# Harshs27/uGLAD

Measured on AMD Instinct MI355X. Metric: GLAD unroll-steps/sec (batch D×D Θ-updates), M=1024 D=128 L=30, higher is better.
Workload: dtype f32; 1 GPU; multi-task M=1024/GPU D=128 L=30 fp32 (BASELINE config 3; global batch 1024); pass=training step: forward + loss + backward + gradient exchange + Adam, sqrt_mode=ns10, parallelism=batch-sharded x1

## Files before the change

uglad_amd/csrc/glad_device.h:

```cpp
#pragma once
#include <hip/hip_runtime.h>

namespace uglad {

#ifndef UGLAD_THREADS
#define UGLAD_THREADS 512
#endif
constexpr int kThreads = UGLAD_THREADS;
constexpr int kWaves = kThreads / 64;
constexpr int kNsIters = 10;

constexpr int P_T = 0, P_RW1 = 1, P_RB1 = 10, P_RW2 = 13, P_RB2 = 22, P_RW3 = 25, P_RB3 = 28;
constexpr int P_LW1 = 29, P_LB1 = 35, P_LW2 = 38, P_LB2 = 41;
constexpr int kNParam = 42, kNRho = 28;

typedef float f32x16 __attribute__((ext_vector_type(16)));
struct alignas(16) f4 {
  float x, y, z, w;
};

#ifdef UGLAD_SIMT_EMUL
#define UGLAD_WAVE_SYNC() simt::wave_sync_point()
#else
#define UGLAD_WAVE_SYNC() asm volatile("s_waitcnt vmcnt(0) lgkmcnt(0)" ::: "memory")
#endif

template <int CTRL, int ROW_MASK = 0xf, int BANK_MASK = 0xf>
__device__ __forceinline__ float dpp_move(float v) {
  return __int_as_float(__builtin_amdgcn_update_dpp(0, __float_as_int(v), CTRL, ROW_MASK, BANK_MASK, false));
}

__device__ __forceinline__ float lane_xor1(float v) { return dpp_move<0xb1>(v); }

__device__ __forceinline__ float sum_halves(float v) {
#ifdef UGLAD_SIMT_EMUL
  return v + __shfl_xor(v, 32);
#else
  const auto r = __builtin_amdgcn_permlane32_swap(__float_as_uint(v), __float_as_uint(v), false, false);
  return __uint_as_float(r[0]) + __uint_as_float(r[1]);
#endif
}

__device__ __forceinline__ int opaque_v(int v) {
#ifndef UGLAD_SIMT_EMUL
  asm volatile("" : "+v"(v));
#endif
  return v;
}

template <typename T>
__device__ __forceinline__ T load_at(const float* __restrict__ base, unsigned bytes) {
  return *reinterpret_cast<const T*>(reinterpret_cast<const char*>(base) + bytes);
}

__device__ __forceinline__ float opaque_f(float v) {
#ifndef UGLAD_SIMT_EMUL
  asm volatile("" : "+v"(v));
#endif
  return v;
}

__device__ __forceinline__ int lane_now() {
#ifdef UGLAD_SIMT_EMUL
  return threadIdx.x & 63;
#else
  int l;
  asm volatile("v_mbcnt_lo_u32_b32 %0, -1, 0\n\tv_mbcnt_hi_u32_b32 %0, -1, %0" : "=v"(l));
  return l;
#endif
}

__device__ __forceinline__ float bcast_lane(float v, int src) {
  return __int_as_float(__builtin_amdgcn_readlane(__float_as_int(v), src));
}

__device__ __forceinline__ float wave_sum(float v) {
  v += dpp_move<0xb1>(v);
  v += dpp_move<0x4e>(v);
  v += dpp_move<0x124>(v);
  v += dpp_move<0x128>(v);
  v += dpp_move<0x142, 0xa>(v);
  v += dpp_move<0x143, 0xc>(v);
  return __int_as_float(__builtin_amdgcn_readlane(__float_as_int(v), 63));
}

__device__ __forceinline__ float block_sum(float v, float* s_red) {
  v = wave_sum(v);
  const int lane = threadIdx.x & 63, w = threadIdx.x >> 6;
  if (lane == 0) s_red[w] = v;
  __syncthreads();
  float t = 0.f;
#pragma unroll
  for (int i = 0; i < kWaves; ++i) t += s_red[i];
  __syncthreads();
  return t;
}

__device__ __forceinline__ float exp_acc(float x) {
  const float t = x * 1.44269504f;
  float e = fmaf(x, 1.44269504f, -t);
  e = fmaf(x, 1.925963033e-8f, e);
  const float r = __builtin_amdgcn_exp2f(t);
  return fmaf(r, e * 0.69314718f, r);
}

__device__ __forceinline__ float div_acc(float a, float b) {
  float q = __builtin_amdgcn_rcpf(b);
  q = fmaf(q, fmaf(-b, q, 1.0f), q);
  return a * q;
}

__device__ __forceinline__ float sigmoidf_(float x) {
  const float t = exp_acc(-fabsf(x));
  const float s = div_acc(1.0f, 1.0f + t);
  return (x >= 0.f) ? s : 1.0f - s;
}

__device__ __forceinline__ float tanhf_(float x) {
  const float t = exp_acc(-2.0f * fabsf(x));
  return copysignf(div_acc(1.0f - t, 1.0f + t), x);
}

struct RhoAct {
  float h1[3], h2[3], rho;
};

__device__ __forceinline__ void rho_forward(const float* __restrict__ p, float x1, float x2, float x3, RhoAct& a) {
#pragma unroll
  for (int o = 0; o < 3; ++o)
    a.h1[o] = tanhf_(fmaf(p[P_RW1 + 3 * o], x1, fmaf(p[P_RW1 + 3 * o + 1], x2, fmaf(p[P_RW1 + 3 * o + 2], x3, p[P_RB1 + o]))));
#pragma unroll
  for (int o = 0; o < 3; ++o)
    a.h2[o] = tanhf_(fmaf(p[P_RW2 + 3 * o], a.h1[0], fmaf(p[P_RW2 + 3 * o + 1], a.h1[1], fmaf(p[P_RW2 + 3 * o + 2], a.h1[2], p[P_RB2 + o]))));
  a.rho = sigmoidf_(fmaf(p[P_RW3], a.h2[0], fmaf(p[P_RW3 + 1], a.h2[1], fmaf(p[P_RW3 + 2], a.h2[2], p[P_RB3]))));
}

typedef float v2f __attribute__((ext_vector_type(2)));
__device__ __forceinline__ v2f fma2(v2f a, v2f b, v2f c) { return __builtin_elementwise_fma(a, b, c); }
__device__ __forceinline__ v2f splat2(float a) { return (v2f){a, a}; }
__device__ __forceinline__ v2f exp_acc2(v2f x) {
  const v2f t = x * 1.44269504f;
  v2f e = fma2(x, splat2(1.44269504f), -t);
  e = fma2(x, splat2(1.925963033e-8f), e);
  const v2f r = {__builtin_amdgcn_exp2f(t.x), __builtin_amdgcn_exp2f(t.y)};
  return fma2(r, e * 0.69314718f, r);
}
__device__ __forceinline__ v2f div_acc2(v2f a, v2f b) {
  v2f q = {__builtin_amdgcn_rcpf(b.x), __builtin_amdgcn_rcpf(b.y)};
  q = fma2(q, fma2(-b, q, splat2(1.0f)), q);
  return a * q;
}
__device__ __forceinline__ v2f tanh2(v2f x) {
  const v2f t = exp_acc2(-2.0f * __builtin_elementwise_abs(x));
  const v2f r = div_acc2(1.0f - t, 1.0f + t);
  return (v2f){copysignf(r.x, x.x), copysignf(r.y, x.y)};
}
__device__ __forceinline__ v2f sigmoid2(v2f x) {
  const v2f t = exp_acc2(-__builtin_elementwise_abs(x));
  const v2f s = div_acc2(splat2(1.0f), 1.0f + t);
  return (v2f){(x.x >= 0.f) ? s.x : 1.0f - s.x, (x.y >= 0.f) ? s.y : 1.0f - s.y};
}
struct RhoAct2 {
  v2f h1[3], h2[3], rho;
  __device__ __forceinline__ RhoAct half(int c) const {
    RhoAct a;
#pragma unroll
    for (int o = 0; o < 3; ++o) {
      a.h1[o] = c ? h1[o].y : h1[o].x;
      a.h2[o] = c ? h2[o].y : h2[o].x;
    }
    a.rho = c ? rho.y : rho.x;
    return a;
  }
};
__device__ __forceinline__ void rho_forward2(const float* __restrict__ p, v2f x1, v2f x2, v2f x3, RhoAct2& a) {
#pragma unroll
  for (int o = 0; o < 3; ++o)
    a.h1[o] = tanh2(fma2(splat2(p[P_RW1 + 3 * o]), x1,
                         fma2(splat2(p[P_RW1 + 3 * o + 1]), x2, fma2(splat2(p[P_RW1 + 3 * o + 2]), x3, splat2(p[P_RB1 + o])))));
#pragma unroll
  for (int o = 0; o < 3; ++o)
    a.h2[o] = tanh2(fma2(splat2(p[P_RW2 + 3 * o]), a.h1[0],
                         fma2(splat2(p[P_RW2 + 3 * o + 1]), a.h1[1], fma2(splat2(p[P_RW2 + 3 * o + 2]), a.h1[2], splat2(p[P_RB2 + o])))));
  a.rho = sigmoid2(fma2(splat2(p[P_RW3]), a.h2[0], fma2(splat2(p[P_RW3 + 1]), a.h2[1], fma2(splat2(p[P_RW3 + 2]), a.h2[2], splat2(p[P_RB3])))));
}

__device__ __forceinline__ float soft_threshold(float x, float rho) {
  const float m = fabsf(x) - rho;
  return m > 0.f ? copysignf(m, x) : 0.f;
}

__device__ __forceinline__ void rho_backward(const float* __restrict__ p, float x1, float x2, float x3, const RhoAct& a,
                                             float g_rho, float w, float* g, float& gx1, float& gx3) {
  const float go = g_rho * a.rho * (1.f - a.rho);
  const float gow = go * w;
  float ga2[3], ga1[3];
#pragma unroll
  for (int h = 0; h < 3; ++h) {
    g[(P_RW3 - 1) + h] += gow * a.h2[h];
    ga2[h] = go * p[P_RW3 + h] * (1.f - a.h2[h] * a.h2[h]);
  }
  g[P_RB3 - 1] += gow;
#pragma unroll
  for (int o = 0; o < 3; ++o) {
    const float t = ga2[o] * w;
#pragma unroll
    for (int h = 0; h < 3; ++h) g[(P_RW2 - 1) + 3 * o + h] += t * a.h1[h];
    g[(P_RB2 - 1) + o] += t;
  }
#pragma unroll
  for (int h = 0; h < 3; ++h) {
    const float s = ga2[0] * p[P_RW2 + h] + ga2[1] * p[P_RW2 + 3 + h] + ga2[2] * p[P_RW2 + 6 + h];
    ga1[h] = s * (1.f - a.h1[h] * a.h1[h]);
  }
#pragma unroll
  for (int o = 0; o < 3; ++o) {
    const float t = ga1[o] * w;
    g[(P_RW1 - 1) + 3 * o + 0] += t * x1;
    g[(P_RW1 - 1) + 3 * o + 1] += t * x2;
    g[(P_RW1 - 1) + 3 * o + 2] += t * x3;
    g[(P_RB1 - 1) + o] += t;
  }
  gx1 = ga1[0] * p[P_RW1 + 0] + ga1[1] * p[P_RW1 + 3] + ga1[2] * p[P_RW1 + 6];
  gx3 = ga1[0] * p[P_RW1 + 2] + ga1[1] * p[P_RW1 + 5] + ga1[2] * p[P_RW1 + 8];
}

__device__ __forceinline__ float rho_backward_col(const float* __restrict__ p, const RhoAct& a, float g_rho, int col) {
  const float go = g_rho * a.rho * (1.f - a.rho);
  float ga2[3], ga1[3];
#pragma unroll
  for (int h = 0; h < 3; ++h) ga2[h] = go * p[P_RW3 + h] * (1.f - a.h2[h] * a.h2[h]);
#pragma unroll
  for (int h = 0; h < 3; ++h) {
    const float s = ga2[0] * p[P_RW2 + h] + ga2[1] * p[P_RW2 + 3 + h] + ga2[2] * p[P_RW2 + 6 + h];
    ga1[h] = s * (1.f - a.h1[h] * a.h1[h]);
  }
  return ga1[0] * p[P_RW1 + col] + ga1[1] * p[P_RW1 + 3 + col] + ga1[2] * p[P_RW1 + 6 + col];
}

__device__ __forceinline__ void rho_backward2(const float* __restrict__ p, v2f x1, v2f x2, v2f x3, const RhoAct2& a, v2f g_rho,
                                              v2f w, v2f* g2, v2f& gx1, v2f& gx3) {
  const v2f go = g_rho * a.rho * (1.f - a.rho);
  const v2f gow = go * w;
  v2f ga2[3], ga1[3];
#pragma unroll
  for (int h = 0; h < 3; ++h) {
    g2[(P_RW3 - 1) + h] = fma2(gow, a.h2[h], g2[(P_RW3 - 1) + h]);
    ga2[h] = go * p[P_RW3 + h] * (1.f - a.h2[h] * a.h2[h]);
  }
  g2[P_RB3 - 1] += gow;
#pragma unroll
  for (int o = 0; o < 3; ++o) {
    const v2f t = ga2[o] * w;
#pragma unroll
    for (int h = 0; h < 3; ++h) g2[(P_RW2 - 1) + 3 * o + h] = fma2(t, a.h1[h], g2[(P_RW2 - 1) + 3 * o + h]);
    g2[(P_RB2 - 1) + o] += t;
  }
#pragma unroll
  for (int h = 0; h < 3; ++h) {
    const v2f s = ga2[0] * p[P_RW2 + h] + ga2[1] * p[P_RW2 + 3 + h] + ga2[2] * p[P_RW2 + 6 + h];
    ga1[h] = s * (1.f - a.h1[h] * a.h1[h]);
  }
#pragma unroll
  for (int o = 0; o < 3; ++o) {
    const v2f t = ga1[o] * w;
    g2[(P_RW1 - 1) + 3 * o + 0] = fma2(t, x1, g2[(P_RW1 - 1) + 3 * o + 0]);
    g2[(P_RW1 - 1) + 3 * o + 1] = fma2(t, x2, g2[(P_RW1 - 1) + 3 * o + 1]);
    g2[(P_RW1 - 1) + 3 * o + 2] = fma2(t, x3, g2[(P_RW1 - 1) + 3 * o + 2]);
    g2[(P_RB1 - 1) + o] += t;
  }
  gx1 = ga1[0] * p[P_RW1 + 0] + ga1[1] * p[P_RW1 + 3] + ga1[2] * p[P_RW1 + 6];
  gx3 = ga1[0] * p[P_RW1 + 2] + ga1[1] * p[P_RW1 + 5] + ga1[2] * p[P_RW1 + 8];
}

__device__ __forceinline__ float lambda_forward(const float* __restrict__ p, float n, float lam_prev) {
  float o = p[P_LB2];
#pragma unroll
  for (int h = 0; h < 3; ++h)
    o = fmaf(p[P_LW2 + h], tanhf(fmaf(p[P_LW1 + 2 * h], n, fmaf(p[P_LW1 + 2 * h + 1], lam_prev, p[P_LB1 + h]))), o);
  return sigmoidf_(o);
}

__device__ __forceinline__ float sqrt_spectrum(float beta, float c, float nrmA, int mode) {
  const float alpha = fmaf(beta, beta, c);
  if (mode == 0) return sqrtf(alpha);
  float y = alpha / nrmA, z = 1.f;
#pragma unroll
  for (int it = 0; it < kNsIters; ++it) {
    const float T = 0.5f * (3.f - z * y);
    y = y * T;
    z = T * z;
  }
  return y * sqrtf(nrmA);
}

__device__ __forceinline__ float shifted_spectrum(float be, int D, float lam, int mode, double* __restrict__ s3, float& alpha,
                                                  float& cond) {
  const int tid = threadIdx.x;
  const double c4 = 4.0 / (double)lam, b = (double)be;
  const double al = b * b + c4;
  const double r_exact = sqrt(al);
  if (tid < D) {
    s3[tid] = al * al;
    s3[D + tid] = 0.5 * (r_exact - b) * b;
    s3[2 * D + tid] = b * b;
  }
  __syncthreads();
  double* part = s3 + 3 * D;
  if ((tid >> 6) == 0) {
    const double* a = s3 + ((tid >> 4) < 3 ? (tid >> 4) : 2) * D;
    double s = 0.0, mx = 0.0, mn = 1e300;
    for (int i = tid & 15; i < D; i += 16) {
      const double v = a[i];
      s += v;
      mx = v > mx ? v : mx;
      mn = v < mn ? v : mn;
    }
#pragma unroll
    for (int o = 1; o < 16; o *= 2) {
      s += __shfl_xor(s, o);
      const double mxo = __shfl_xor(mx, o), mno = __shfl_xor(mn, o);
      mx = mxo > mx ? mxo : mx;
      mn = mno < mn ? mno : mn;
    }
    if ((tid & 15) == 0 && tid < 48) part[tid >> 4] = s;
    if (tid == 32) {
      part[3] = mx;
      part[4] = mn;
    }
  }
  __syncthreads();
  const double n2 = part[0], pb = part[1], bb = part[2], b2max = part[3], b2min = part[4];
  cond = (float)((b2max + c4) / (b2min + c4));
  double a_opt = (bb > 0.0) ? -pb / bb : 0.0;
  a_opt = a_opt < 0.0 ? 0.0 : (a_opt > 1.0 ? 1.0 : a_opt);
  alpha = (float)a_opt;
  double r = r_exact;
  if (mode != 0) {
    const double nrmA = sqrt(n2);
    double y = al / nrmA, z = 1.0;
#pragma unroll
    for (int it = 0; it < kNsIters; ++it) {
      const double T = 0.5 * (3.0 - z * y);
      y = y * T;
      z = T * z;
    }
    r = y * sqrt(nrmA);
  }
  const double psi = 0.5 * (r - b) + (double)alpha * b;
  __syncthreads();
  return (tid < D) ? (float)psi : 0.f;
}

template <int DP>
__device__ __forceinline__ void pair_of(int r, int k, int& i1, int& i2) {
  constexpr int m = DP - 1;
  if (k == 0) {
    i1 = m;
    i2 = r;
  } else {
    i1 = r + k;
    if (i1 >= m) i1 -= m;
    i2 = r + m - k;
    if (i2 >= m) i2 -= m;
  }
}

template <int DP>
__device__ void jacobi_eig(float* __restrict__ A, float* __restrict__ V, float* s_t, float* s_s, float* s_h, float* s_red,
                           int* s_flag) {
  constexpr int LD = DP + 1, H = DP / 2;
  const int tid = threadIdx.x;
  float fro = 0.f;
  for (int idx = tid; idx < DP * DP; idx += kThreads) {
    const float v = A[(idx / DP) * LD + (idx % DP)];
    fro = fmaf(v, v, fro);
  }
  fro = sqrtf(block_sum(fro, s_red));
  const float thresh = 1e-8f * fro;
  for (int sweep = 0; sweep < 16; ++sweep) {
    if (tid == 0) *s_flag = 0;
    __syncthreads();
    for (int r = 0; r < DP - 1; ++r) {
      if (tid < H) {
        int p, q;
        pair_of<DP>(r, tid, p, q);
        const float apq = A[p * LD + q];
        float t = 0.f, s = 0.f, h = 0.f;
        if (fabsf(apq) > thresh) {
          const float app = A[p * LD + p], aqq = A[q * LD + q];
          const float tau = (aqq - app) / (2.f * apq);
          t = copysignf(1.f, tau) / (fabsf(tau) + sqrtf(fmaf(tau, tau, 1.f)));
          const float c = 1.f / sqrtf(fmaf(t, t, 1.f));
          s = t * c;
          h = s / (1.f + c);
          *s_flag = 1;
        }
        s_t[tid] = t;
        s_s[tid] = s;
        s_h[tid] = h;
      }
      __syncthreads();
      for (int b = tid; b < H * H; b += kThreads) {
        const int kr = b / H, kc = b - kr * H;
        int r1, r2, c1, c2;
        pair_of<DP>(r, kr, r1, r2);
        pair_of<DP>(r, kc, c1, c2);
        const float x11 = A[r1 * LD + c1], x12 = A[r1 * LD + c2], x21 = A[r2 * LD + c1], x22 = A[r2 * LD + c2];
        float z11, z12, z21, z22;
        if (kr == kc) {
          const float t = s_t[kr];
          z11 = x11 - t * x12;
          z22 = x22 + t * x12;
          z12 = (t != 0.f) ? 0.f : x12;
          z21 = (t != 0.f) ? 0.f : x21;
        } else {
          const float sr = s_s[kr], hr = s_h[kr], sc = s_s[kc], hc = s_h[kc];
          const float y11 = x11 - sr * (x21 + hr * x11), y21 = x21 + sr * (x11 - hr * x21);
          const float y12 = x12 - sr * (x22 + hr * x12), y22 = x22 + sr * (x12 - hr * x22);
          z11 = y11 - sc * (y12 + hc * y11);
          z12 = y12 + sc * (y11 - hc * y12);
          z21 = y21 - sc * (y22 + hc * y21);
          z22 = y22 + sc * (y21 - hc * y22);
        }
        A[r1 * LD + c1] = z11;
        A[r1 * LD + c2] = z12;
        A[r2 * LD + c1] = z21;
        A[r2 * LD + c2] = z22;
      }
      for (int b = tid; b < DP * H; b += kThreads) {
        const int i = b / H, kc = b - i * H;
        int c1, c2;
        pair_of<DP>(r, kc, c1, c2);
        const float sc = s_s[kc], hc = s_h[kc];
        const float v1 = V[i * LD + c1], v2 = V[i * LD + c2];
        V[i * LD + c1] = v1 - sc * (v2 + hc * v1);
        V[i * LD + c2] = v2 + sc * (v1 - hc * v2);
      }
      __syncthreads();
    }
    if (*s_flag == 0) break;
    __syncthreads();
  }
  __syncthreads();
}

template <int NT, bool UPPER>
struct Tiles {
  static constexpr int kCount = UPPER ? NT * (NT + 1) / 2 : NT * NT;
  static constexpr int kPerWave = (kCount + kWaves - 1) / kWaves;
  __device__ static __forceinline__ void ij(int t, int& I, int& J) {
    if (UPPER) {
      int i = 0, rem = t;
      while (rem >= NT - i) {
        rem -= NT - i;
        ++i;
      }
      I = i;
      J = i + rem;
    } else {
      I = t / NT;
      J = t - I * NT;
    }
  }
};

__device__ __forceinline__ int acc_row(int reg, int lane) { return (reg & 3) + 8 * (reg >> 2) + 4 * (lane >> 5); }

__device__ __forceinline__ void mfma_tile(const float* __restrict__ Ap, int a_si, int a_sk, const float* __restrict__ Bp,
                                          int b_sk, int b_sj, int K, f32x16& acc) {
  const int lane = opaque_v(threadIdx.x) & 63, li = lane & 31, kh = lane >> 5;
  const float* a = Ap + li * a_si + kh * a_sk;
  const float* b = Bp + li * b_sj + kh * b_sk;
  float a0[8], b0[8], a1[8], b1[8];
#pragma unroll
  for (int u = 0; u < 8; ++u) {
    a0[u] = a[2 * u * a_sk];
    b0[u] = b[2 * u * b_sk];
  }
  for (int k = 0; k < K; k += 16) {
    const bool more = k + 16 < K;
    const float* an = a + (more ? 16 * a_sk : 0);
    const float* bn = b + (more ? 16 * b_sk : 0);
#pragma unroll
    for (int u = 0; u < 8; ++u) {
      a1[u] = an[2 * u * a_sk];
      b1[u] = bn[2 * u * b_sk];
    }
#pragma unroll
    for (int u = 0; u < 8; ++u) acc = __builtin_amdgcn_mfma_f32_32x32x2f32(a0[u], b0[u], acc, 0, 0, 0);
#pragma unroll
    for (int u = 0; u < 8; ++u) {
      a0[u] = a1[u];
      b0[u] = b1[u];
    }
    a = an;
    b = bn;
  }
}

#if defined(UGLAD_BF16X3) && !defined(UGLAD_SIMT_EMUL)
#include "../../scripts/retired/bf16x3_tile.h"
#define UGLAD_GEMM_TILE mfma_tile_bf16x3
#else
#define UGLAD_GEMM_TILE mfma_tile
#endif

template <int NT, bool TA, bool TB, bool UPPER>
__device__ __forceinline__ void gemm_lds(const float* __restrict__ X, const float* __restrict__ Y,
                                         f32x16 (&acc)[Tiles<NT, UPPER>::kPerWave]) {
  constexpr int DP = NT * 32, LD = DP + 1;
  using T = Tiles<NT, UPPER>;
  const int w = __builtin_amdgcn_readfirstlane(opaque_v(threadIdx.x) >> 6);
#pragma unroll
  for (int n = 0; n < T::kPerWave; ++n) {
    const int t = w + kWaves * n;
#pragma unroll
    for (int e = 0; e < 16; ++e) acc[n][e] = 0.f;
    if (t < T::kCount) {
      int I, J;
      T::ij(t, I, J);
      UGLAD_GEMM_TILE(TA ? X + I * 32 : X + I * 32 * LD, TA ? 1 : LD, TA ? LD : 1, TB ? Y + J * 32 * LD : Y + J * 32,
                      TB ? 1 : LD, TB ? LD : 1, DP, acc[n]);
    }
  }
}

template <int NT>
__device__ __forceinline__ void store_tiles(float* __restrict__ Y, const f32x16 (&acc)[Tiles<NT, false>::kPerWave]) {
  constexpr int LD = NT * 32 + 1;
  using T = Tiles<NT, false>;
  const int tid = opaque_v(threadIdx.x), lane = tid & 63, w = __builtin_amdgcn_readfirstlane(tid >> 6);
#pragma unroll
  for (int n = 0; n < T::kPerWave; ++n) {
    const int t = w + kWaves * n;
    if (t < T::kCount) {
      int I, J;
      T::ij(t, I, J);
#pragma unroll
      for (int e = 0; e < 16; ++e) Y[(I * 32 + acc_row(e, lane)) * LD + J * 32 + (lane & 31)] = acc[n][e];
    }
  }
}

#ifdef UGLAD_STAMPS
__device__ unsigned long long g_cwg[4096][3];
__device__ unsigned long long g_lstamps[4][96];
__device__ unsigned long long g_kstamps[32];
#define KSTAMP(i) do { if (threadIdx.x == 0 && blockIdx.x == 0) g_kstamps[i] = __builtin_amdgcn_s_memtime(); } while (0)
#define UGLAD_STAMP(ws, i) do { if (threadIdx.x == 0 && (i) < 64) (ws).stamp[i] = __builtin_amdgcn_s_memtime(); } while (0)
#elif defined(UGLAD_PHASE_EXIT)
__device__ int g_exit_at;
#define KSTAMP(i) do { if (g_exit_at == 100 + (i)) __builtin_amdgcn_endpgm(); } while (0)
#define UGLAD_STAMP(ws, i) do { if (g_exit_at == (i)) __builtin_amdgcn_endpgm(); } while (0)
#else
#define KSTAMP(i) do {} while (0)
#define UGLAD_STAMP(ws, i) do {} while (0)
#endif

__device__ __forceinline__ void copy_out_matrix(float* __restrict__ dst, const float* __restrict__ src, int D, int LD) {
  const int tid = threadIdx.x;
  if (((D & 3) == 0) && ((reinterpret_cast<size_t>(dst) & 15) == 0)) {
    const int D4 = D >> 2;
    for (int idx = tid; idx < D * D4; idx += kThreads) {
      const int i = idx / D4, j = 4 * (idx - i * D4);
      const float* p = src + i * LD + j;
      f4 v = {p[0], p[1], p[2], p[3]};
      *reinterpret_cast<f4*>(dst + (size_t)i * D + j) = v;
    }
  } else {
    const int si = kThreads / D, sj = kThreads - si * D;
    int i = tid / D, j = tid - i * D;
    for (int idx = tid; idx < D * D; idx += kThreads) {
      dst[idx] = src[i * LD + j];
      j += sj;
      i += si;
      if (j >= D) {
        j -= D;
        ++i;
      }
    }
  }
}

template <int DP>
constexpr int kTfacFloats = (DP / 32) * 1024;
template <int DP>
constexpr int kWsPerMatrix = 3 * DP + kTfacFloats<DP>;
template <int DP>
constexpr int big_floats() {
  return 2 * ((DP * (DP + 1) + 3) & ~3);
}
#define UGLAD_BIG_BUFFERS(A, NA, B, NB, GWS)                                                                     \
  constexpr bool kGM = DP > 128;                                                                                 \
  __shared__ __attribute__((aligned(16))) float A##_lds[kGM ? 4 : (NA)];                                         \
  __shared__ __attribute__((aligned(16))) float B##_lds[kGM ? 4 : (NB)];                                         \
  float* A = kGM ? (GWS) + (size_t)gridDim.x * kWsPerMatrix<DP> + (size_t)blockIdx.x * big_floats<DP>() : A##_lds; \
  float* B = kGM ? A + big_floats<DP>() / 2 : B##_lds;

template <int DP>
__device__ __forceinline__ float* tfac_behind_flags(float* ws, int M, int m) {
  static_assert(kTfacFloats<DP> / 2 >= 4, "flags and packed T factors outgrow the T region: M + 3 <= M kTfacFloats / 2 needs kTfacFloats / 2 >= 4");
  return ws + (size_t)M * 3 * DP + ((M + 3) & ~3) + (size_t)m * (kTfacFloats<DP> / 2);
}

}
```

uglad_amd/csrc/tridiag.h:

```cpp
#pragma once
#include "glad_device.h"

namespace uglad {

constexpr float kNegligibleSig = 1e-35f;

#ifdef UGLAD_STAMPS
__device__ unsigned long long g_tstamps[4];
__device__ unsigned long long g_twg[4096][3];
#define TSTAMP_BEGIN() const unsigned long long t_begin_ = __builtin_amdgcn_s_memtime()
#define TSTAMP_ADD(i) do { if (threadIdx.x == 0 && blockIdx.x == 0) g_tstamps[i] += __builtin_amdgcn_s_memtime() - t_begin_; } while (0)
#else
#define TSTAMP_BEGIN() do {} while (0)
#define TSTAMP_ADD(i) do {} while (0)
#endif

__device__ __forceinline__ float f4_elem(const f4& a, int q) { return q == 0 ? a.x : (q == 1 ? a.y : (q == 2 ? a.z : a.w)); }

template <int N>
__device__ __forceinline__ float pick(const float (&v)[N], int idx) {
  float r = v[0];
#pragma unroll
  for (int s = 1; s < N; ++s) r = (idx == s) ? v[s] : r;
  return r;
}

template <int NT, int TH>
__global__ __launch_bounds__(TH, NT <= 4 ? 8 : (TH > 512 ? 1 : 2)) void tridiag_kernel(const float* __restrict__ A0, const float* __restrict__ A1,
                                                           const float* __restrict__ lam_ptr, float* __restrict__ Rbase,
                                                           float* __restrict__ tri_base, int D, int gs,
                                                           const int* __restrict__ only_flagged) {
  if (only_flagged && only_flagged[blockIdx.x] == 0) return;
  constexpr int DP = NT * 32, RG = DP / 4, NCG = TH / RG, NC = (DP + NCG - 1) / NCG;
  constexpr int NS = (DP > 128) ? (DP + 63) / 64 : 2;
  constexpr int NL = (NT == 4 && TH == 512) ? 3 : 0;
  __shared__ f4 s_a[NL > 0 ? NL : 1][NL > 0 ? TH : 1];
  __shared__ __attribute__((aligned(16))) float s_vec[5 * DP];
#ifndef UGLAD_TRIDIAG_ROWWAVES
#define UGLAD_TRIDIAG_ROWWAVES 0
#endif
#ifndef UGLAD_TRIDIAG_PRIO
#define UGLAD_TRIDIAG_PRIO 1
#endif
#ifndef UGLAD_TRIDIAG_PAIRSUM
#define UGLAD_TRIDIAG_PAIRSUM 0
#endif
#ifndef UGLAD_TRIDIAG_LANE
#define UGLAD_TRIDIAG_LANE 0
#endif
#ifndef UGLAD_TRIDIAG_DPPSUM
#define UGLAD_TRIDIAG_DPPSUM 0
#endif
  constexpr bool kDppSum = UGLAD_TRIDIAG_DPPSUM && !UGLAD_TRIDIAG_ROWWAVES && (NT == 4 && TH == 512);
  constexpr bool kRowWaves = UGLAD_TRIDIAG_ROWWAVES && (NT == 4 && TH == 512);
  constexpr bool kPairSum = UGLAD_TRIDIAG_PAIRSUM && !kRowWaves && RG == 32 && (NCG % 2 == 0);
  constexpr int NPG = kDppSum ? 1 : (kPairSum ? NCG / 2 : NCG);
  constexpr int PS = kRowWaves ? DP + 4 : DP;
  __shared__ __attribute__((aligned(16))) float s_part[kRowWaves ? (TH / (DP / 4)) * (DP + 4) : TH * 4];
  __shared__ float s_dotp[(TH / 64)];
  __shared__ float s_corner, s_tau;
  const int tid = threadIdx.x, lane = tid & 63, wv = tid >> 6;
  const int wv_u = __builtin_amdgcn_readfirstlane(wv);
#ifdef UGLAD_STAMPS
  if (tid == 0 && blockIdx.x < 4096) {
    g_twg[blockIdx.x][0] = __builtin_amdgcn_s_memtime();
    unsigned hw, xcc;
    asm volatile("s_getreg_b32 %0, hwreg(HW_REG_HW_ID)" : "=s"(hw));
    asm volatile("s_getreg_b32 %0, hwreg(HW_REG_XCC_ID)" : "=s"(xcc));
    g_twg[blockIdx.x][2] = ((unsigned long long)xcc << 32) | hw;
  }
#endif
  const int r4 = kDppSum ? wv + 8 * (lane >> 4) : (kRowWaves ? 4 * wv + (lane & 3) : tid % RG);
  const int cg = kDppSum ? (lane & 15) : (kRowWaves ? lane >> 2 : tid / RG);
  const int cgw = (kRowWaves || kDppSum) ? NCG - 1 : (__builtin_amdgcn_readfirstlane(wv) * 64 + 63) / RG;
  const int cgmax = cgw < NCG - 1 ? cgw : NCG - 1;
  const int row_last = kRowWaves ? 16 * __builtin_amdgcn_readfirstlane(wv) + 15 : DP;
  const int n = D;
  const size_t base = (size_t)blockIdx.x * D * D;
  float* R = Rbase + base;
  float* tri = tri_base + (size_t)blockIdx.x * 3 * DP;
  const float inv_lam = lam_ptr ? 1.0f / lam_ptr[blockIdx.x / gs] : 1.0f;

  f4 a[NC];
  {
    auto pin = [](float v) { return opaque_f(v); };
    constexpr int LB = 4, LS = (NT == 3) ? 1 : 2;
    const float* __restrict__ Am = A0 + base;
    const float* __restrict__ Zm = A1 ? A1 + base : nullptr;
    const bool vec16 = !kDppSum && ((D & 3) == 0) && (((reinterpret_cast<size_t>(A0) | reinterpret_cast<size_t>(A1)) & 15) == 0);
    if (vec16) {
      const bool row_in = cg < NCG && 4 * r4 < n;
#pragma unroll
      for (int i0 = 0; i0 < NC; i0 += LB) {
        f4 s[LB], z[LB];
#pragma unroll
        for (int u = 0; u < LB; ++u) {
          const int c = cg + NCG * (i0 + u);
          const unsigned at = (i0 + u < NC && row_in && c < n) ? 4u * (c * D + 4 * r4) : 0u;
          s[u] = load_at<f4>(Am, at);
        }
        if (A1) {
#pragma unroll
          for (int u = 0; u < LB; ++u) {
            const int c = cg + NCG * (i0 + u);
            const unsigned at = (i0 + u < NC && row_in && c < n) ? 4u * (c * D + 4 * r4) : 0u;
            z[u] = load_at<f4>(Zm, at);
          }
          __builtin_amdgcn_sched_barrier(0);
        }
#pragma unroll
        for (int u = 0; u < LB; ++u) {
          const int i = i0 + u;
          if (i < NC) {
            const bool in = row_in && cg + NCG * i < n;
            f4 v = s[u];
            if (A1) v = {fmaf(inv_lam, v.x, -z[u].x), fmaf(inv_lam, v.y, -z[u].y), fmaf(inv_lam, v.z, -z[u].z), fmaf(inv_lam, v.w, -z[u].w)};
            a[i] = {pin(in ? v.x : 0.f), pin(in ? v.y : 0.f), pin(in ? v.z : 0.f), pin(in ? v.w : 0.f)};
            if (i < NL) s_a[i < NL ? i : 0][tid] = a[i];
          }
        }
      }
    } else {
#pragma unroll
      for (int i0 = 0; i0 < NC; i0 += LS) {
        float s[LS][4], z[LS][4];
#pragma unroll
        for (int u = 0; u < LS; ++u) {
          const int c = cg + NCG * (i0 + u);
#pragma unroll
          for (int q = 0; q < 4; ++q) {
            const int r = 4 * r4 + q;
            const bool in = i0 + u < NC && cg < NCG && c < n && r < n;
            const unsigned at = in ? 4u * (kDppSum ? r * D + c : c * D + r) : 0u;
            s[u][q] = load_at<float>(Am, at);
          }
        }
        if (A1) {
#pragma unroll
          for (int u = 0; u < LS; ++u) {
            const int c = cg + NCG * (i0 + u);
#pragma unroll
            for (int q = 0; q < 4; ++q) {
              const int r = 4 * r4 + q;
              const bool in = i0 + u < NC && cg < NCG && c < n && r < n;
              const unsigned at = in ? 4u * (kDppSum ? r * D + c : c * D + r) : 0u;
              z[u][q] = load_at<float>(Zm, at);
            }
          }
        }
#pragma unroll
        for (int u = 0; u < LS; ++u) {
          const int i = i0 + u;
          if (i < NC) {
            float t[4];
#pragma unroll
            for (int q = 0; q < 4; ++q) {
              const bool in = cg < NCG && cg + NCG * i < n && 4 * r4 + q < n;
              float v = s[u][q];
              if (A1) v = fmaf(inv_lam, v, -z[u][q]);
              t[q] = pin(in ? v : 0.f);
            }
            a[i] = {t[0], t[1], t[2], t[3]};
            if (i < NL) s_a[i < NL ? i : 0][tid] = a[i];
          }
        }
        __builtin_amdgcn_sched_barrier(0);
      }
    }
  }
  for (int i = tid; i < DP; i += TH) {
    s_vec[i] = 0.f;
    s_vec[DP + i] = 0.f;
    s_vec[2 * DP + i] = 0.f;
    tri[i] = 0.f;
    tri[DP + i] = 0.f;
    tri[2 * DP + i] = 0.f;
  }
  for (int i = tid; i < (int)(sizeof(s_part) / sizeof(float)); i += TH) s_part[i] = 0.f;
  if (tid < (TH / 64)) s_dotp[tid] = 0.f;
  if (cg == 0) *reinterpret_cast<f4*>(&s_vec[3 * DP + 4 * r4]) = a[0];
  if (cg < NCG && r4 == ((n - 1) >> 2)) {
#pragma unroll
    for (int i = 0; i < NC; ++i)
      if (cg + NCG * i == n - 1) s_corner = f4_elem(a[i], (n - 1) & 3);
  }
  __syncthreads();
  if (n == 1) {
    if (tid == 0) tri[0] = s_corner;
    return;
  }

#ifdef UGLAD_STAMPS
  if (tid == 0 && blockIdx.x == 0) g_tstamps[2] += __builtin_amdgcn_s_memtime() - g_twg[0][0];
#endif
  int ov = DP, on = 2 * DP;
  float tau_k = 0.f;
  int cur = 0;
  for (int k = -1; k <= n - 3; ++k) {
    const int k1 = k + 1;
    {
    TSTAMP_BEGIN();
    if (wv_u == 0) {
      if (UGLAD_TRIDIAG_PRIO) __builtin_amdgcn_s_setprio(3);
#if UGLAD_TRIDIAG_LANE == 1
      const int lane = lane_now();
      const int lane_k = lane;
#elif UGLAD_TRIDIAG_LANE == 2
      const int lane_k = lane_now();
#else
      const int lane_k = lane;
#endif
      float pv[NS], vv[NS], wl[NS];
#pragma unroll
      for (int s = 0; s < NS; ++s) {
        const int rr = lane_k + 64 * s;
        float p = 0.f;
        if (rr > k && lane + 64 * s < n) {
#pragma unroll 8
          for (int g = 0; g < NPG; ++g) p += s_part[g * PS + rr];
          p *= tau_k;
        }
        pv[s] = p;
        vv[s] = (lane + 64 * s < DP) ? s_vec[ov + rr] : 0.f;
      }
      float vAv2[2] = {0.f, 0.f};
#pragma unroll
      for (int q = 0; q < (TH / 64); ++q) vAv2[q & 1] += s_dotp[q];
      const float vAv = vAv2[0] + vAv2[1];
      const float alpha = 0.5f * tau_k * tau_k * vAv;
#pragma unroll
      for (int s = 0; s < NS; ++s) {
        const int rr = lane_k + 64 * s;
        wl[s] = pv[s] - alpha * vv[s];
        if (lane + 64 * s < DP) s_vec[rr] = wl[s];
      }
      const float w_k1 = bcast_lane(pick(wl, k1 >> 6), k1 & 63);
      const float v_k1 = bcast_lane(pick(vv, k1 >> 6), k1 & 63);
      float x[NS];
#pragma unroll
      for (int s = 0; s < NS; ++s) {
        const int c = lane_k + 64 * s;
        x[s] = (lane + 64 * s < n) ? (s_vec[(3 + cur) * DP + c] - v_k1 * wl[s] - w_k1 * vv[s]) : 0.f;
      }
      const float dk1 = bcast_lane(pick(x, k1 >> 6), k1 & 63);
      if (k1 <= n - 3) {
        const int c0 = k1 + 1;
        const float x0 = bcast_lane(pick(x, c0 >> 6), c0 & 63);
        float sig = 0.f;
#pragma unroll
        for (int s = 0; s < NS; ++s) {
          const int c = lane_k + 64 * s;
          if (c > c0 && lane + 64 * s < n) sig = fmaf(x[s], x[s], sig);
        }
        sig = wave_sum(sig);
        float beta = x0, tau1 = 0.f, sc = 0.f;
        if (sig > kNegligibleSig) {
          const float nrm2 = fmaf(x0, x0, sig);
          if (nrm2 > 1e-30f) {
            beta = -copysignf(__builtin_amdgcn_sqrtf(nrm2), x0);
            const float dd = x0 - beta;
            sc = div_acc(1.0f, dd);
            tau1 = -dd * div_acc(1.0f, beta);
          } else {
            beta = -copysignf(sqrtf(nrm2), x0);
            tau1 = (beta - x0) / beta;
            sc = 1.0f / (x0 - beta);
          }
        }
#pragma unroll
        for (int s = 0; s < NS; ++s) {
          const int c = lane_k + 64 * s;
          if (lane + 64 * s < DP) {
            float vc = 0.f;
            if (c == c0) vc = 1.f;
            else if (c > c0 && lane + 64 * s < n) vc = x[s] * sc;
            s_vec[on + c] = vc;
            if (lane + 64 * s < n) R[(size_t)k1 * D + c] = vc;
          }
        }
        if (lane == 0) {
          tri[k1] = dk1;
          tri[DP + k1] = beta;
          tri[2 * DP + k1] = tau1;
          s_tau = tau1;
        }
      } else {
        const float e_last = bcast_lane(pick(x, (n - 1) >> 6), (n - 1) & 63);
        const float w_n1 = bcast_lane(pick(wl, (n - 1) >> 6), (n - 1) & 63);
        const float v_n1 = bcast_lane(pick(vv, (n - 1) >> 6), (n - 1) & 63);
        if (lane == 0) {
          tri[k1] = dk1;
          tri[DP + k1] = e_last;
          tri[n - 1] = s_corner - 2.f * v_n1 * w_n1;
        }
      }
      if (UGLAD_TRIDIAG_PRIO) __builtin_amdgcn_s_setprio(0);
    }
    __syncthreads();
    TSTAMP_ADD(0);
    }
    if (k1 > n - 3) break;
    tau_k = s_tau;
    TSTAMP_BEGIN();
    float vav = 0.f;
    const int k2 = k1 + 1;
    if (cg < NCG) {
      f4 acc = {0.f, 0.f, 0.f, 0.f};
      const float* vr = s_vec + 4 * r4;
      const float* vcol = s_vec + cg;
      const f4 v4 = *reinterpret_cast<const f4*>(vr + ov);
      const f4 w4 = *reinterpret_cast<const f4*>(vr);
      constexpr int PB = (NT > 4) ? 8 : 1;
#pragma unroll
      for (int i0 = 0; i0 < NC; i0 += PB) {
        if (cgmax + NCG * (i0 + PB - 1) > k1 && row_last > k) {
          float vcv[PB], wcv[PB], ncv[PB];
#pragma unroll
          for (int u = 0; u < PB; ++u) {
            const int cc = cg + NCG * (i0 + u);
            const int c = ((NCG * NC > DP && cc >= DP) || i0 + u >= NC) ? 0 : cc;
            const int co = c - cg;
            vcv[u] = vcol[ov + co];
            wcv[u] = vcol[co];
            ncv[u] = vcol[on + co];
          }
#pragma unroll
          for (int u = 0; u < PB; ++u) {
            const int i = i0 + u;
            if (i < NC && cgmax + NCG * i > k1) {
              const float vc = vcv[u], wc = wcv[u], nc = ncv[u];
              f4 t = (i < NL) ? s_a[i < NL ? i : 0][tid] : a[i < NC ? i : 0];
              t.x = t.x - vc * w4.x - wc * v4.x;
              t.y = t.y - vc * w4.y - wc * v4.y;
              t.z = t.z - vc * w4.z - wc * v4.z;
              t.w = t.w - vc * w4.w - wc * v4.w;
              acc.x = fmaf(t.x, nc, acc.x);
              acc.y = fmaf(t.y, nc, acc.y);
              acc.z = fmaf(t.z, nc, acc.z);
              acc.w = fmaf(t.w, nc, acc.w);
              if (i < NL) s_a[i < NL ? i : 0][tid] = t;
              else a[i < NC ? i : 0] = t;
            }
          }
        }
      }
      const f4 n4 = *reinterpret_cast<const f4*>(vr + on);
      vav = acc.x * n4.x + acc.y * n4.y + acc.z * n4.z + acc.w * n4.w;
      if (kDppSum) {
        acc.x += dpp_move<0xb1>(acc.x); acc.y += dpp_move<0xb1>(acc.y); acc.z += dpp_move<0xb1>(acc.z); acc.w += dpp_move<0xb1>(acc.w);
        acc.x += dpp_move<0x4e>(acc.x); acc.y += dpp_move<0x4e>(acc.y); acc.z += dpp_move<0x4e>(acc.z); acc.w += dpp_move<0x4e>(acc.w);
        acc.x += dpp_move<0x124>(acc.x); acc.y += dpp_move<0x124>(acc.y); acc.z += dpp_move<0x124>(acc.z); acc.w += dpp_move<0x124>(acc.w);
        acc.x += dpp_move<0x128>(acc.x); acc.y += dpp_move<0x128>(acc.y); acc.z += dpp_move<0x128>(acc.z); acc.w += dpp_move<0x128>(acc.w);
        if (cg == 0) *reinterpret_cast<f4*>(&s_part[4 * r4]) = acc;
      } else if (kPairSum) {
        acc.x = sum_halves(acc.x);
        acc.y = sum_halves(acc.y);
        acc.z = sum_halves(acc.z);
        acc.w = sum_halves(acc.w);
        if (lane < 32) *reinterpret_cast<f4*>(&s_part[(cg >> 1) * PS + 4 * r4]) = acc;
      } else {
        *reinterpret_cast<f4*>(&s_part[cg * PS + 4 * r4]) = acc;
      }
      const int i2 = k2 / NCG;
      if (cg == k2 - i2 * NCG) {
        f4* dst = reinterpret_cast<f4*>(s_vec + 4 * r4 + (3 + (cur ^ 1)) * DP);
#pragma unroll
        for (int i = 0; i < NC; ++i)
          if (i2 == i) *dst = (i < NL) ? s_a[i < NL ? i : 0][tid] : a[i];
      }
      if (k1 == n - 3) {
        const int ic = (n - 1) / NCG;
        if (cg == (n - 1) - ic * NCG && r4 == ((n - 1) >> 2)) {
#pragma unroll
          for (int i = 0; i < NC; ++i)
            if (ic == i) s_corner = f4_elem((i < NL) ? s_a[i < NL ? i : 0][tid] : a[i], (n - 1) & 3);
        }
      }
    }
    vav = wave_sum(vav);
#if UGLAD_TRIDIAG_LANE == 0
    if (lane == 0) s_dotp[wv] = vav;
#else
    if (lane_now() == 0) s_dotp[wv_u] = vav;
#endif
    __syncthreads();
    TSTAMP_ADD(1);
    const int t = ov;
    ov = on;
    on = t;
    cur ^= 1;
  }
#ifdef UGLAD_STAMPS
  if (tid == 0 && blockIdx.x < 4096) g_twg[blockIdx.x][1] = __builtin_amdgcn_s_memtime();
#endif
}

}
```

Before: 1.228 million unroll-steps/s.

## Restructure tridiag leader-wave reduction, stage outputs in LDS, vectorize Householder row writes

```diff
diff --git a/uglad_amd/csrc/glad_device.h b/uglad_amd/csrc/glad_device.h
--- a/uglad_amd/csrc/glad_device.h
+++ b/uglad_amd/csrc/glad_device.h
@@ -58,16 +58,6 @@
   asm volatile("" : "+v"(v));
 #endif
   return v;
-}
-
-__device__ __forceinline__ int lane_now() {
-#ifdef UGLAD_SIMT_EMUL
-  return threadIdx.x & 63;
-#else
-  int l;
-  asm volatile("v_mbcnt_lo_u32_b32 %0, -1, 0\n\tv_mbcnt_hi_u32_b32 %0, -1, %0" : "=v"(l));
-  return l;
-#endif
 }
 
 __device__ __forceinline__ float bcast_lane(float v, int src) {
diff --git a/uglad_amd/csrc/tridiag.h b/uglad_amd/csrc/tridiag.h
--- a/uglad_amd/csrc/tridiag.h
+++ b/uglad_amd/csrc/tridiag.h
@@ -21,7 +21,7 @@
 __device__ __forceinline__ float pick(const float (&v)[N], int idx) {
   float r = v[0];
 #pragma unroll
-  for (int s = 1; s < N; ++s) r = (idx == s) ? v[s] : r;
+  for (int s = 1; s < N; ++s) r = (idx == s) ? (N > 3 ? opaque_f(v[s]) : v[s]) : r;
   return r;
 }
 
@@ -33,30 +33,16 @@
   if (only_flagged && only_flagged[blockIdx.x] == 0) return;
   constexpr int DP = NT * 32, RG = DP / 4, NCG = TH / RG, NC = (DP + NCG - 1) / NCG;
   constexpr int NS = (DP > 128) ? (DP + 63) / 64 : 2;
+  constexpr int kPadR = 64 * NS - DP;
   constexpr int NL = (NT == 4 && TH == 512) ? 3 : 0;
   __shared__ f4 s_a[NL > 0 ? NL : 1][NL > 0 ? TH : 1];
-  __shared__ __attribute__((aligned(16))) float s_vec[5 * DP];
-#ifndef UGLAD_TRIDIAG_ROWWAVES
-#define UGLAD_TRIDIAG_ROWWAVES 0
-#endif
+  __shared__ __attribute__((aligned(16))) float s_vec[5 * DP + kPadR];
 #ifndef UGLAD_TRIDIAG_PRIO
 #define UGLAD_TRIDIAG_PRIO 1
 #endif
-#ifndef UGLAD_TRIDIAG_PAIRSUM
-#define UGLAD_TRIDIAG_PAIRSUM 0
-#endif
-#ifndef UGLAD_TRIDIAG_LANE
-#define UGLAD_TRIDIAG_LANE 0
-#endif
-#ifndef UGLAD_TRIDIAG_DPPSUM
-#define UGLAD_TRIDIAG_DPPSUM 0
-#endif
-  constexpr bool kDppSum = UGLAD_TRIDIAG_DPPSUM && !UGLAD_TRIDIAG_ROWWAVES && (NT == 4 && TH == 512);
-  constexpr bool kRowWaves = UGLAD_TRIDIAG_ROWWAVES && (NT == 4 && TH == 512);
-  constexpr bool kPairSum = UGLAD_TRIDIAG_PAIRSUM && !kRowWaves && RG == 32 && (NCG % 2 == 0);
-  constexpr int NPG = kDppSum ? 1 : (kPairSum ? NCG / 2 : NCG);
-  constexpr int PS = kRowWaves ? DP + 4 : DP;
-  __shared__ __attribute__((aligned(16))) float s_part[kRowWaves ? (TH / (DP / 4)) * (DP + 4) : TH * 4];
+  constexpr int NPG = NCG;
+  __shared__ __attribute__((aligned(16))) float s_part[TH * 4 + kPadR];
+  __shared__ float s_tri[3 * DP];
   __shared__ float s_dotp[(TH / 64)];
   __shared__ float s_corner, s_tau;
   const int tid = threadIdx.x, lane = tid & 63, wv = tid >> 6;
@@ -70,11 +56,9 @@
     g_twg[blockIdx.x][2] = ((unsigned long long)xcc << 32) | hw;
   }
 #endif
-  const int r4 = kDppSum ? wv + 8 * (lane >> 4) : (kRowWaves ? 4 * wv + (lane & 3) : tid % RG);
-  const int cg = kDppSum ? (lane & 15) : (kRowWaves ? lane >> 2 : tid / RG);
-  const int cgw = (kRowWaves || kDppSum) ? NCG - 1 : (__builtin_amdgcn_readfirstlane(wv) * 64 + 63) / RG;
+  const int r4 = tid % RG, cg = tid / RG;
+  const int cgw = (__builtin_amdgcn_readfirstlane(wv) * 64 + 63) / RG;
   const int cgmax = cgw < NCG - 1 ? cgw : NCG - 1;
-  const int row_last = kRowWaves ? 16 * __builtin_amdgcn_readfirstlane(wv) + 15 : DP;
   const int n = D;
   const size_t base = (size_t)blockIdx.x * D * D;
   float* R = Rbase + base;
@@ -87,7 +71,7 @@
     constexpr int LB = 4, LS = (NT == 3) ? 1 : 2;
     const float* __restrict__ Am = A0 + base;
     const float* __restrict__ Zm = A1 ? A1 + base : nullptr;
-    const bool vec16 = !kDppSum && ((D & 3) == 0) && (((reinterpret_cast<size_t>(A0) | reinterpret_cast<size_t>(A1)) & 15) == 0);
+    const bool vec16 = ((D & 3) == 0) && (((reinterpret_cast<size_t>(A0) | reinterpret_cast<size_t>(A1)) & 15) == 0);
     if (vec16) {
       const bool row_in = cg < NCG && 4 * r4 < n;
 #pragma unroll
@@ -131,7 +115,7 @@
           for (int q = 0; q < 4; ++q) {
             const int r = 4 * r4 + q;
             const bool in = i0 + u < NC && cg < NCG && c < n && r < n;
-            const unsigned at = in ? 4u * (kDppSum ? r * D + c : c * D + r) : 0u;
+            const unsigned at = in ? 4u * (c * D + r) : 0u;
             s[u][q] = load_at<float>(Am, at);
           }
         }
@@ -143,7 +127,7 @@
             for (int q = 0; q < 4; ++q) {
               const int r = 4 * r4 + q;
               const bool in = i0 + u < NC && cg < NCG && c < n && r < n;
-              const unsigned at = in ? 4u * (kDppSum ? r * D + c : c * D + r) : 0u;
+              const unsigned at = in ? 4u * (c * D + r) : 0u;
               z[u][q] = load_at<float>(Zm, at);
             }
           }
@@ -172,9 +156,9 @@
     s_vec[i] = 0.f;
     s_vec[DP + i] = 0.f;
     s_vec[2 * DP + i] = 0.f;
-    tri[i] = 0.f;
-    tri[DP + i] = 0.f;
-    tri[2 * DP + i] = 0.f;
+    s_tri[i] = 0.f;
+    s_tri[DP + i] = 0.f;
+    s_tri[2 * DP + i] = 0.f;
   }
   for (int i = tid; i < (int)(sizeof(s_part) / sizeof(float)); i += TH) s_part[i] = 0.f;
   if (tid < (TH / 64)) s_dotp[tid] = 0.f;
@@ -185,10 +169,7 @@
       if (cg + NCG * i == n - 1) s_corner = f4_elem(a[i], (n - 1) & 3);
   }
   __syncthreads();
-  if (n == 1) {
-    if (tid == 0) tri[0] = s_corner;
-    return;
-  }
+  if (n == 1 && tid == 0) s_tri[0] = s_corner;
 
 #ifdef UGLAD_STAMPS
   if (tid == 0 && blockIdx.x == 0) g_tstamps[2] += __builtin_amdgcn_s_memtime() - g_twg[0][0];
@@ -196,52 +177,88 @@
   int ov = DP, on = 2 * DP;
   float tau_k = 0.f;
   int cur = 0;
+  const bool r16 = ((D & 3) == 0) && ((reinterpret_cast<size_t>(Rbase) & 15) == 0);
   for (int k = -1; k <= n - 3; ++k) {
     const int k1 = k + 1;
     {
     TSTAMP_BEGIN();
     if (wv_u == 0) {
       if (UGLAD_TRIDIAG_PRIO) __builtin_amdgcn_s_setprio(3);
-#if UGLAD_TRIDIAG_LANE == 1
-      const int lane = lane_now();
-      const int lane_k = lane;
-#elif UGLAD_TRIDIAG_LANE == 2
-      const int lane_k = lane_now();
-#else
-      const int lane_k = lane;
-#endif
+      constexpr int G0 = (NS == 2) ? 2 : 1;
+      constexpr int GB = (NS == 2) ? 7 : (TH == 1024 ? 5 : 12 / NS);
+      constexpr bool kEarly = TH != 1024;
+      bool in_n[NS];
+      float vraw[NS], xraw[NS], dot[TH / 64];
+#pragma unroll
+      for (int s = 0; s < NS; ++s) {
+        const int rr = lane + 64 * s;
+        in_n[s] = 64 * s < DP && rr < n;
+        if (kEarly) {
+          vraw[s] = (64 * s < DP) ? s_vec[ov + lane + 64 * s] : 0.f;
+          xraw[s] = (64 * s < DP) ? s_vec[(3 + cur) * DP + lane + 64 * s] : 0.f;
+        }
+      }
+      auto sum_dot = [&]() __attribute__((always_inline)) {
+#pragma unroll
+        for (int q = 0; q < (TH / 64); ++q) dot[q] = s_dotp[q];
+        float vAv2[2] = {0.f, 0.f};
+#pragma unroll
+        for (int q = 0; q < (TH / 64); ++q) vAv2[q & 1] += dot[q];
+        return vAv2[0] + vAv2[1];
+      };
       float pv[NS], vv[NS], wl[NS];
+      auto gather = [&](const int g0, const int cnt) __attribute__((always_inline)) {
+        float pq[GB > G0 ? GB : G0][NS];
+#pragma unroll
+        for (int u = 0; u < cnt; ++u) {
+          const int g = (g0 + u < NPG) ? g0 + u : 0;
+#pragma unroll
+          for (int s = 0; s < NS; ++s) pq[u][s] = (64 * s < DP) ? s_part[g * DP + lane + 64 * s] : 0.f;
+        }
+#pragma unroll
+        for (int u = 0; u < cnt; ++u) {
+          if (g0 + u < NPG) {
+#pragma unroll
+            for (int s = 0; s < NS; ++s) pv[s] += pq[u][s];
+          }
+        }
+      };
+#pragma unroll
+      for (int s = 0; s < NS; ++s) pv[s] = 0.f;
+      float vAv = 0.f;
+      if (kEarly) vAv = sum_dot();
+      gather(0, G0);
+      constexpr int kGatherUnroll = (NPG - G0 <= 2 * GB) ? 2 : 1;
+#pragma unroll kGatherUnroll
+      for (int g0 = G0; g0 < NPG; g0 += GB) {
+        __builtin_amdgcn_sched_barrier(0);
+        gather(g0, GB);
+      }
+      if (!kEarly) {
+        __builtin_amdgcn_sched_barrier(0);
+#pragma unroll
+        for (int s = 0; s < NS; ++s) {
+          vraw[s] = (64 * s < DP) ? s_vec[ov + lane + 64 * s] : 0.f;
+          xraw[s] = (64 * s < DP) ? s_vec[(3 + cur) * DP + lane + 64 * s] : 0.f;
+        }
+        vAv = sum_dot();
+      }
+      const float alpha = 0.5f * tau_k * tau_k * vAv;
 #pragma unroll
       for (int s = 0; s < NS; ++s) {
-        const int rr = lane_k + 64 * s;
-        float p = 0.f;
-        if (rr > k && lane + 64 * s < n) {
-#pragma unroll 8
-          for (int g = 0; g < NPG; ++g) p += s_part[g * PS + rr];
-          p *= tau_k;
-        }
-        pv[s] = p;
-        vv[s] = (lane + 64 * s < DP) ? s_vec[ov + rr] : 0.f;
-      }
-      float vAv2[2] = {0.f, 0.f};
-#pragma unroll
-      for (int q = 0; q < (TH / 64); ++q) vAv2[q & 1] += s_dotp[q];
-      const float vAv = vAv2[0] + vAv2[1];
-      const float alpha = 0.5f * tau_k * tau_k * vAv;
+        pv[s] = (in_n[s] && lane + 64 * s > k) ? pv[s] * tau_k : 0.f;
+        vv[s] = (lane + 64 * s < DP) ? vraw[s] : 0.f;
+      }
 #pragma unroll
       for (int s = 0; s < NS; ++s) {
-        const int rr = lane_k + 64 * s;
         wl[s] = pv[s] - alpha * vv[s];
-        if (lane + 64 * s < DP) s_vec[rr] = wl[s];
+        if (lane + 64 * s < DP) s_vec[lane + 64 * s] = wl[s];
       }
       const float w_k1 = bcast_lane(pick(wl, k1 >> 6), k1 & 63);
       const float v_k1 = bcast_lane(pick(vv, k1 >> 6), k1 & 63);
       float x[NS];
 #pragma unroll
-      for (int s = 0; s < NS; ++s) {
-        const int c = lane_k + 64 * s;
-        x[s] = (lane + 64 * s < n) ? (s_vec[(3 + cur) * DP + c] - v_k1 * wl[s] - w_k1 * vv[s]) : 0.f;
-      }
+      for (int s = 0; s < NS; ++s) x[s] = in_n[s] ? (xraw[s] - opaque_f(v_k1 * wl[s]) - opaque_f(w_k1 * vv[s])) : 0.f;
       const float dk1 = bcast_lane(pick(x, k1 >> 6), k1 & 63);
       if (k1 <= n - 3) {
         const int c0 = k1 + 1;
@@ -249,14 +266,14 @@
         float sig = 0.f;
 #pragma unroll
         for (int s = 0; s < NS; ++s) {
-          const int c = lane_k + 64 * s;
-          if (c > c0 && lane + 64 * s < n) sig = fmaf(x[s], x[s], sig);
+          const float xs = (lane + 64 * s > c0) ? x[s] : 0.f;
+          sig = fmaf(xs, xs, sig);
         }
         sig = wave_sum(sig);
         float beta = x0, tau1 = 0.f, sc = 0.f;
-        if (sig > kNegligibleSig) {
+        if (__builtin_expect(sig > kNegligibleSig, 1)) {
           const float nrm2 = fmaf(x0, x0, sig);
-          if (nrm2 > 1e-30f) {
+          if (__builtin_expect(nrm2 > 1e-30f, 1)) {
             beta = -copysignf(__builtin_amdgcn_sqrtf(nrm2), x0);
             const float dd = x0 - beta;
             sc = div_acc(1.0f, dd);
@@ -269,19 +286,14 @@
         }
 #pragma unroll
         for (int s = 0; s < NS; ++s) {
-          const int c = lane_k + 64 * s;
-          if (lane + 64 * s < DP) {
-            float vc = 0.f;
-            if (c == c0) vc = 1.f;
-            else if (c > c0 && lane + 64 * s < n) vc = x[s] * sc;
-            s_vec[on + c] = vc;
-            if (lane + 64 * s < n) R[(size_t)k1 * D + c] = vc;
-          }
+          const int c = lane + 64 * s;
+          const float vc = (c == c0) ? 1.f : ((c > c0 && in_n[s]) ? x[s] * sc : 0.f);
+          if (c < DP) s_vec[on + c] = vc;
         }
         if (lane == 0) {
-          tri[k1] = dk1;
-          tri[DP + k1] = beta;
-          tri[2 * DP + k1] = tau1;
+          s_tri[k1] = dk1;
+          s_tri[DP + k1] = beta;
+          s_tri[2 * DP + k1] = tau1;
           s_tau = tau1;
         }
       } else {
@@ -289,9 +301,9 @@
         const float w_n1 = bcast_lane(pick(wl, (n - 1) >> 6), (n - 1) & 63);
         const float v_n1 = bcast_lane(pick(vv, (n - 1) >> 6), (n - 1) & 63);
         if (lane == 0) {
-          tri[k1] = dk1;
-          tri[DP + k1] = e_last;
-          tri[n - 1] = s_corner - 2.f * v_n1 * w_n1;
+          s_tri[k1] = dk1;
+          s_tri[DP + k1] = e_last;
+          s_tri[n - 1] = s_corner - 2.f * v_n1 * w_n1;
         }
       }
       if (UGLAD_TRIDIAG_PRIO) __builtin_amdgcn_s_setprio(0);
@@ -306,14 +318,17 @@
     const int k2 = k1 + 1;
     if (cg < NCG) {
       f4 acc = {0.f, 0.f, 0.f, 0.f};
+      f4* const sa = &s_a[0][0] + (NL > 0 ? opaque_v(tid) : 0);
       const float* vr = s_vec + 4 * r4;
       const float* vcol = s_vec + cg;
       const f4 v4 = *reinterpret_cast<const f4*>(vr + ov);
       const f4 w4 = *reinterpret_cast<const f4*>(vr);
+      const int dead = k1 - cgmax;
+      const int i_first = dead < 0 ? 0 : dead / NCG + 1;
       constexpr int PB = (NT > 4) ? 8 : 1;
 #pragma unroll
       for (int i0 = 0; i0 < NC; i0 += PB) {
-        if (cgmax + NCG * (i0 + PB - 1) > k1 && row_last > k) {
+        if (i0 + PB - 1 >= i_first) {
           float vcv[PB], wcv[PB], ncv[PB];
 #pragma unroll
           for (int u = 0; u < PB; ++u) {
@@ -327,9 +342,9 @@
 #pragma unroll
           for (int u = 0; u < PB; ++u) {
             const int i = i0 + u;
-            if (i < NC && cgmax + NCG * i > k1) {
+            if (i < NC && i >= i_first) {
               const float vc = vcv[u], wc = wcv[u], nc = ncv[u];
-              f4 t = (i < NL) ? s_a[i < NL ? i : 0][tid] : a[i < NC ? i : 0];
+              f4 t = (i < NL) ? sa[(i < NL ? i : 0) * TH] : a[i < NC ? i : 0];
               t.x = t.x - vc * w4.x - wc * v4.x;
               t.y = t.y - vc * w4.y - wc * v4.y;
               t.z = t.z - vc * w4.z - wc * v4.z;
@@ -338,51 +353,43 @@
               acc.y = fmaf(t.y, nc, acc.y);
               acc.z = fmaf(t.z, nc, acc.z);
               acc.w = fmaf(t.w, nc, acc.w);
-              if (i < NL) s_a[i < NL ? i : 0][tid] = t;
+              if (i < NL) sa[(i < NL ? i : 0) * TH] = t;
               else a[i < NC ? i : 0] = t;
             }
           }
         }
       }
       const f4 n4 = *reinterpret_cast<const f4*>(vr + on);
-      vav = acc.x * n4.x + acc.y * n4.y + acc.z * n4.z + acc.w * n4.w;
-      if (kDppSum) {
-        acc.x += dpp_move<0xb1>(acc.x); acc.y += dpp_move<0xb1>(acc.y); acc.z += dpp_move<0xb1>(acc.z); acc.w += dpp_move<0xb1>(acc.w);
-        acc.x += dpp_move<0x4e>(acc.x); acc.y += dpp_move<0x4e>(acc.y); acc.z += dpp_move<0x4e>(acc.z); acc.w += dpp_move<0x4e>(acc.w);
-        acc.x += dpp_move<0x124>(acc.x); acc.y += dpp_move<0x124>(acc.y); acc.z += dpp_move<0x124>(acc.z); acc.w += dpp_move<0x124>(acc.w);
-        acc.x += dpp_move<0x128>(acc.x); acc.y += dpp_move<0x128>(acc.y); acc.z += dpp_move<0x128>(acc.z); acc.w += dpp_move<0x128>(acc.w);
-        if (cg == 0) *reinterpret_cast<f4*>(&s_part[4 * r4]) = acc;
-      } else if (kPairSum) {
-        acc.x = sum_halves(acc.x);
-        acc.y = sum_halves(acc.y);
-        acc.z = sum_halves(acc.z);
-        acc.w = sum_halves(acc.w);
-        if (lane < 32) *reinterpret_cast<f4*>(&s_part[(cg >> 1) * PS + 4 * r4]) = acc;
-      } else {
-        *reinterpret_cast<f4*>(&s_part[cg * PS + 4 * r4]) = acc;
-      }
-      const int i2 = k2 / NCG;
-      if (cg == k2 - i2 * NCG) {
+      vav = fmaf(acc.w, n4.w, fmaf(acc.z, n4.z, fmaf(acc.x, n4.x, acc.y * n4.y)));
+      *reinterpret_cast<f4*>(&s_part[cg * DP + 4 * r4]) = acc;
+      const int i2 = k2 / NCG, cg2 = k2 - i2 * NCG;
+      if (cg == cg2) {
         f4* dst = reinterpret_cast<f4*>(s_vec + 4 * r4 + (3 + (cur ^ 1)) * DP);
 #pragma unroll
         for (int i = 0; i < NC; ++i)
-          if (i2 == i) *dst = (i < NL) ? s_a[i < NL ? i : 0][tid] : a[i];
+          if (i2 == i) *dst = (i < NL) ? sa[(i < NL ? i : 0) * TH] : a[i];
+      }
+      if (cg == (cg2 > 0 ? cg2 - 1 : NCG - 1)) {
+        float* Rrow = R + (size_t)k1 * D + 4 * (opaque_v(tid) % RG);
+        if (r16) {
+          if (4 * r4 < n) *reinterpret_cast<f4*>(Rrow) = n4;
+        } else {
+#pragma unroll
+          for (int q = 0; q < 4; ++q)
+            if (4 * r4 + q < n) Rrow[q] = f4_elem(n4, q);
+        }
       }
       if (k1 == n - 3) {
         const int ic = (n - 1) / NCG;
         if (cg == (n - 1) - ic * NCG && r4 == ((n - 1) >> 2)) {
 #pragma unroll
           for (int i = 0; i < NC; ++i)
-            if (ic == i) s_corner = f4_elem((i < NL) ? s_a[i < NL ? i : 0][tid] : a[i], (n - 1) & 3);
+            if (ic == i) s_corner = f4_elem((i < NL) ? sa[(i < NL ? i : 0) * TH] : a[i], opaque_v((n - 1) & 3));
         }
       }
     }
     vav = wave_sum(vav);
-#if UGLAD_TRIDIAG_LANE == 0
     if (lane == 0) s_dotp[wv] = vav;
-#else
-    if (lane_now() == 0) s_dotp[wv_u] = vav;
-#endif
     __syncthreads();
     TSTAMP_ADD(1);
     const int t = ov;
@@ -390,6 +397,7 @@
     on = t;
     cur ^= 1;
   }
+  for (int i = tid; i < 3 * DP; i += TH) tri[i] = s_tri[i];
 #ifdef UGLAD_STAMPS
   if (tid == 0 && blockIdx.x < 4096) g_twg[blockIdx.x][1] = __builtin_amdgcn_s_memtime();
 #endif
```

Result: faster. 1.254 million unroll-steps/s, median of 6 (+2.1%).
